# lowc1012/tensorflow-distributed-example

Hardware: AMD Instinct MI355X
Metric: images/sec (whole node) MNIST CNN at 1/2/4/8 MI355X; step time ms (higher is better)
Workload: dtype fp32; 1 GPU; model=mnist_cnn, global_batch=64, per_gpu_batch=64, parallelism=dp1, replicas=1, replicas_per_process=1, distinct_devices=1, graphs_per_execution=1, steps_per_execution=3, warmup_steps_run=6783, optimizer=SGD(lr=0.001), plan=fused_convnet, allreduce=none, hipgraph=True, grad_buckets=1, optimizer_placement=in_step_kernels

## Files before the change

### csrc/include/tde_convnet.h

```cpp
#pragma once
#include "tde_optim.h"
#include "tde_xgmi.h"

namespace tde {
namespace cnet {

constexpr int CC = 32;
constexpr int HD = 64;
constexpr int NW = 16;

struct FwdArgs {
  const float* x; const float* wc; const float* bc;
  const void* W1; int ldw1;
  float* hpre;
  void* Pt; int ldPt;
  uint64_t* amax; int lda;
  int B, H, W;
  long long* stamps;
  int w1_rows;
  const int* pend;
  const float *gwc, *gbc, *mwc, *mbc, *vwc, *vbc;
  const long long* iterations;
  OptHyper h;
  unsigned long long* inc_iter;
// ... 137 lines not shown
    for (int t = 0; t < 9; ++t) {
      wlo[t] = *reinterpret_cast<const float4*>(wcs + t * CC + c0);
      whi[t] = *reinterpret_cast<const float4*>(wcs + t * CC + c0 + 4);
    }
    blo = *reinterpret_cast<const float4*>(wcs + 9 * CC + c0);
    bhi = *reinterpret_cast<const float4*>(wcs + 9 * CC + c0 + 4);
  }
};

__device__ __forceinline__ float f4get(float4 q, int k) { return k == 0 ? q.x : (k == 1 ? q.y : (k == 2 ? q.z : q.w)); }

__device__ __forceinline__ void conv_pool8(const float* xb, int W, const ConvW8& cw, float out[8], uint64_t& packed) {
  float patch[16];
#pragma unroll
  for (int r = 0; r < 4; ++r) {
    const float2 u = *reinterpret_cast<const float2*>(xb + r * W);
    const float2 v = *reinterpret_cast<const float2*>(xb + r * W + 2);
    patch[r * 4 + 0] = u.x; patch[r * 4 + 1] = u.y; patch[r * 4 + 2] = v.x; patch[r * 4 + 3] = v.y;
  }
  packed = 0;
#pragma unroll
  for (int cc = 0; cc < 8; ++cc) {
    float wt[9];
#pragma unroll
    for (int t = 0; t < 9; ++t) wt[t] = f4get(cc < 4 ? cw.wlo[t] : cw.whi[t], cc & 3);
    const float bcv = f4get(cc < 4 ? cw.blo : cw.bhi, cc & 3);
    float best = -3.0e38f;
    int bi = 0;
#pragma unroll
    for (int q = 0; q < 4; ++q) {
      const int dy = q >> 1, dx = q & 1;
      float z = bcv;
#pragma unroll
      for (int ky = 0; ky < 3; ++ky)
#pragma unroll
        for (int kx = 0; kx < 3; ++kx) z = fmaf(patch[(dy + ky) * 4 + dx + kx], wt[ky * 3 + kx], z);
      if (z > best) { best = z; bi = q; }
    }
    out[cc] = fmaxf(best, 0.f);
    packed |= (uint64_t)(best > 0.f ? (unsigned)bi : 0xFFu) << (8 * cc);
  }
}

struct BwdArgs {
  const float* x; const uint64_t* amax; int lda;
  const float* hpre;
  float* hzero;
  int hrep; long long hrep_stride;
  float* cpart;
  const float* b1; const float* W2; const float* b2; int C; int pre_relu;
  const int* labels;
  float scale;
  float* metrics;
  const void* W1; int ldw1;
  const void* Pt; int ldPt;
  float* dW1;
  float* dwc; float* dbc;
  int crep; long long crep_stride;
  float *dW2, *db2, *db1;
  int B, H, W;
  long long* stamps;
  float *w1, *m1, *v1;
  bf16* w1r_out;
  bf16* w1c_out; int ldw1c;
  float *hw, *hm, *hv;
  long long off_w2, off_b2, off_b1;
  const long long* iterations;
  long long* iter_prev;
  OptHyper h;
  FlatApply commit;
  int* pend_set;
  XgPush push;
};

template <int NPER>
struct FlatPrefetch {
  int e[NPER];
  float w[NPER], g[NPER], m[NPER], v[NPER];
  __device__ __forceinline__ void load(const FlatApply& f, int tid, int nt) {
#pragma unroll
    for (int k = 0; k < NPER; ++k) {
      int idx = tid + k * nt;
      e[k] = -1;
      for (int r = 0; r < f.nr; ++r) {
        if (idx < f.n[r]) {
          e[k] = f.lo[r] + idx;
          break;
        }
        idx -= f.n[r];
      }
      w[k] = g[k] = m[k] = v[k] = 0.f;
      if (e[k] >= 0) {
        w[k] = f.w[e[k]];
        g[k] = flat_grad(f, e[k]);
        if (opt_has_m(f.h.kind)) m[k] = f.m[e[k]];
        if (opt_has_v(f.h.kind)) v[k] = f.v[e[k]];
      }
    }
  }
  __device__ __forceinline__ void apply(const FlatApply& f, long long t) {
    const float lr_t = opt_lr_t(f.h, t);
#pragma unroll
    for (int k = 0; k < NPER; ++k) {
      if (e[k] < 0) continue;
      f.w[e[k]] = opt_step(f.h, lr_t, w[k], g[k], m[k], v[k]);
      flat_grad_zero(f, e[k]);
      if (opt_has_m(f.h.kind)) f.m[e[k]] = m[k];
      if (opt_has_v(f.h.kind)) f.v[e[k]] = v[k];
    }
  }
};

__device__ __forceinline__ f32x4 mfma_f32x4(float a, float b, f32x4 c) {
  return __builtin_amdgcn_mfma_f32_16x16x4f32(a, b, c, 0, 0, 0);
}

constexpr int HS = HD + 4;
constexpr int DLS = 17, W2S = 17;
constexpr int kHeadScratch = 64 * HS * 4 + 12 * 64 * 4 * 4 + 64 * DLS * 4;
struct HeadLds {
  float* hs;
  float* part;
  float* dls;
  float* w2s;
  float* b2s;
  int* labs;
  __device__ __forceinline__ static HeadLds carve(unsigned char* scratch, unsigned char* w2, unsigned char* b2,
                                                  unsigned char* lab) {
    HeadLds l;
    l.hs = reinterpret_cast<float*>(scratch);
    l.part = reinterpret_cast<float*>(scratch + 64 * HS * 4);
    l.dls = reinterpret_cast<float*>(scratch + 64 * HS * 4 + 12 * 64 * 4 * 4);
    l.w2s = reinterpret_cast<float*>(w2);
    l.b2s = reinterpret_cast<float*>(b2);
    l.labs = reinterpret_cast<int*>(lab);
    return l;
  }
};
constexpr int kW2Bytes = HD * W2S * 4, kB2Bytes = 16 * 4, kLabBytes = 64 * 4;

__device__ __forceinline__ void head_load_w2(const BwdArgs& a, const HeadLds& l, int tid) {
  const int u = tid >> 4, c = tid & 15;
  l.w2s[u * W2S + c] = c < a.C ? a.W2[u * a.C + c] : 0.f;
  if (tid < 16) l.b2s[tid] = tid < a.C ? a.b2[tid] : 0.f;
}

__device__ __forceinline__ void zero_other_parity(const BwdArgs& a, int tid) {
  const int n4 = (int)(((a.hrep - 1) * a.hrep_stride + (long long)a.B * HD) / 4);
  const int per = (n4 + gridDim.x - 1) / gridDim.x, beg = blockIdx.x * per;
  const int end = min(n4, beg + per);
  for (int i = beg + tid; i < end; i += 1024) reinterpret_cast<float4*>(a.hzero)[i] = float4{0.f, 0.f, 0.f, 0.f};
}

__device__ __forceinline__ int opaque_tid() {
  int t = threadIdx.x;
  asm volatile("" : "+v"(t));
  return t;
}

constexpr int kMaxRep = 8;
template <int N>
struct HpreRep {
  float4 v[N];
  __device__ __forceinline__ void issue(const BwdArgs& a, int row, int c4) {
#pragma unroll
    for (int r = 0; r < N; ++r)
      v[r] = *reinterpret_cast<const float4*>(a.hpre + (size_t)min(r, a.hrep - 1) * a.hrep_stride + (size_t)row * HD + c4);
  }
  __device__ __forceinline__ float4 sum(const BwdArgs& a) const {
    float4 s = v[0];
#pragma unroll
    for (int r = 1; r < N; ++r) {
      const bool on = r < a.hrep;
      s.x += on ? v[r].x : 0.f; s.y += on ? v[r].y : 0.f; s.z += on ? v[r].z : 0.f; s.w += on ? v[r].w : 0.f;
    }
    return s;
  }
};
__device__ __forceinline__ float4 load_hpre_loop(const BwdArgs& a, int row, int c4) {
  float4 s = {0.f, 0.f, 0.f, 0.f};
  for (int r = 0; r < a.hrep; ++r) {
    const float4 v = *reinterpret_cast<const float4*>(a.hpre + (size_t)r * a.hrep_stride + (size_t)row * HD + c4);
    s.x += v.x; s.y += v.y; s.z += v.z; s.w += v.w;
  }
  return s;
}
template <int N>
__device__ __forceinline__ float4 load_hpre_n(const BwdArgs& a, int row, int c4) {
  HpreRep<N> h;
  h.issue(a, row, c4);
  return h.sum(a);
}
__device__ __forceinline__ float4 load_hpre_sw(const BwdArgs& a, int row, int c4) {
  if (a.hrep > kMaxRep) return load_hpre_loop(a, row, c4);
  switch (a.hrep) {
    case 1: return load_hpre_n<1>(a, row, c4);
    case 2: return load_hpre_n<2>(a, row, c4);
    case 3: case 4: return load_hpre_n<4>(a, row, c4);
    default: return load_hpre_n<8>(a, row, c4);
  }
}
__device__ __forceinline__ float4 load_hpre(const BwdArgs& a, int row, int c4) {
  if (a.hrep > kMaxRep) return load_hpre_loop(a, row, c4);
  float4 v[kMaxRep];
#pragma unroll
  for (int r = 0; r < kMaxRep; ++r)
    v[r] = r < a.hrep ? *reinterpret_cast<const float4*>(a.hpre + (size_t)r * a.hrep_stride + (size_t)row * HD + c4)
                      : float4{0.f, 0.f, 0.f, 0.f};
  float4 s = v[0];
#pragma unroll
  for (int r = 1; r < kMaxRep; ++r) {
    s.x += v[r].x; s.y += v[r].y; s.z += v[r].z; s.w += v[r].w;
  }
  return s;
}

__device__ __forceinline__ void head_stage(const BwdArgs& a, float4 hv, float4 b1v, int hr, int hc4, int nb,
                                           float* hs) {
  float4 h = float4{hv.x + b1v.x, hv.y + b1v.y, hv.z + b1v.z, hv.w + b1v.w};
  if (a.pre_relu) h = float4{fmaxf(h.x, 0.f), fmaxf(h.y, 0.f), fmaxf(h.z, 0.f), fmaxf(h.w, 0.f)};
  if (hr >= nb) h = float4{0.f, 0.f, 0.f, 0.f};
  *reinterpret_cast<float4*>(hs + hr * HS + hc4) = h;
}

__device__ __forceinline__ void head_logits_ce(const BwdArgs& a, int nb, const HeadLds& l, int lane, int wave,
                                               float& la, float& ca, float& na) {
  const int fr = lane & 15, fq = lane >> 4, C = a.C;
  f32x4 lg = {0.f, 0.f, 0.f, 0.f};
  {
    const int rt = wave & 3, kq = wave >> 2;
#pragma unroll
    for (int k = kq * 16; k < kq * 16 + 16; k += 4)
      lg = mfma_f32x4(l.hs[(rt * 16 + fr) * HS + k + fq], l.w2s[(k + fq) * W2S + fr], lg);
    if (kq > 0) *reinterpret_cast<f32x4*>(l.part + (((kq - 1) * 4 + rt) * 64 + lane) * 4) = lg;
  }
  lds_barrier();
  if (wave < 4) {
    const int rt = wave;
#pragma unroll
    for (int q = 0; q < 3; ++q) {
      const f32x4 pv = *reinterpret_cast<const f32x4*>(l.part + ((q * 4 + rt) * 64 + lane) * 4);
      lg[0] += pv[0]; lg[1] += pv[1]; lg[2] += pv[2]; lg[3] += pv[3];
    }
#pragma unroll
    for (int i = 0; i < 4; ++i) {
      const int r = rt * 16 + fq * 4 + i;
      const bool valid = r < nb;
      const bool cv = fr < C;
      const float z = cv ? lg[i] + l.b2s[fr] : -3.0e38f;
      const float m = row16_max(z);
      const float e = cv ? __expf(z - m) : 0.f;
      const float s = row16_sum(e);
      const float pr = e / s;
      const int label = l.labs[r];
      const int amx = row16_min(cv && z == m ? fr : 64);
      const float zl = __shfl(z, (lane & ~15) | (label & 15), 64);
      if (valid && fr == 0) {
        la += __logf(s) + m - zl;
        ca += (amx == label) ? 1.f : 0.f;
        na += 1.f;
      }
      l.dls[r * DLS + fr] = (valid && cv) ? (pr - (fr == label ? 1.f : 0.f)) * a.scale : 0.f;
    }
  }
  lds_barrier();
}

__device__ __forceinline__ f32x4 head_dh(const BwdArgs& a, int nb, const HeadLds& l, int lane, int wave) {
  const int fr = lane & 15, fq = lane >> 4, rt = wave >> 2, ut = wave & 3;
  f32x4 gh = {0.f, 0.f, 0.f, 0.f};
#pragma unroll
  for (int k = 0; k < 16; k += 4)
    gh = mfma_f32x4(l.dls[(rt * 16 + fr) * DLS + k + fq], l.w2s[(ut * 16 + fr) * W2S + k + fq], gh);
  const int j = ut * 16 + fr;
#pragma unroll
  for (int i = 0; i < 4; ++i) {
    const int r = rt * 16 + fq * 4 + i;
    if ((a.pre_relu && !(l.hs[r * HS + j] > 0.f)) || r >= nb) gh[i] = 0.f;
  }
  return gh;
}

__device__ __forceinline__ long long head_var(const BwdArgs& a, int tid, int i) {
  const int lane = tid & 63, wave = tid >> 6, fr = lane & 15, fq = lane >> 4, C = a.C;
  if (wave < 4 && fr < C) return a.off_w2 + (long long)(wave * 16 + fq * 4 + i) * C + fr;
  if (i == 0 && wave == 4 && fq == 0 && fr < C) return a.off_b2 + fr;
  if (i == 0 && wave == 5 && a.off_b1 >= 0) return a.off_b1 + lane;
  return -1;
}

template <int MODE, bool LEAN = false>
__device__ __forceinline__ void head_workgroup(const BwdArgs& a, const HeadLds& l, float* db1p) {
  const int lane = threadIdx.x & 63, wave = threadIdx.x >> 6, tid = threadIdx.x;
  const int fr = lane & 15, fq = lane >> 4, C = a.C;
  const float4 b1v = a.b1 ? *reinterpret_cast<const float4*>(a.b1 + (tid & 15) * 4) : float4{0.f, 0.f, 0.f, 0.f};

  float hwv[4] = {0.f, 0.f, 0.f, 0.f}, hmv[4] = {0.f, 0.f, 0.f, 0.f}, hvv[4] = {0.f, 0.f, 0.f, 0.f};
  long long t_it = 0;
  FlatPrefetch<1> cp;
  int cpend = 0;
  if (MODE != 0) {
    t_it = *a.iterations;
    const int tl = LEAN ? opaque_tid() : (int)threadIdx.x;
#pragma unroll
    for (int i = 0; i < 4; ++i) {
      const long long e = head_var(a, tl, i);
      if (e < 0) continue;
      hwv[i] = a.hw[e];
      if (MODE == 2 && opt_has_m(a.h.kind)) hmv[i] = a.hm[e];
      if (MODE == 2 && opt_has_v(a.h.kind)) hvv[i] = a.hv[e];
    }
    if (a.commit.nr > 0) {
      cpend = *a.commit.pend;
      cp.load(a.commit, tid, 1024);
    }
  }

  f32x4 gw = {0.f, 0.f, 0.f, 0.f};
  float db1acc = 0.f, db2acc = 0.f, la = 0.f, ca = 0.f, na = 0.f;
  for (int b0 = 0; b0 < a.B; b0 += 64) {
    const int nb = min(64, a.B - b0);
    const int tid = LEAN ? opaque_tid() : (int)threadIdx.x;
    const int lane = tid & 63, wave = tid >> 6, fr = lane & 15, fq = lane >> 4;
    const int hr = tid >> 4, hc4 = (tid & 15) * 4;
    float4 hv = {0.f, 0.f, 0.f, 0.f};
    if (hr < nb) hv = LEAN ? load_hpre_sw(a, b0 + hr, hc4) : load_hpre(a, b0 + hr, hc4);
    const int lab = (tid < nb) ? a.labels[b0 + tid] : 0;
    head_stage(a, hv, b1v, hr, hc4, nb, l.hs);
    if (tid < 64) l.labs[tid] = lab;
    lds_barrier();
    head_logits_ce(a, nb, l, lane, wave, la, ca, na);
    const f32x4 gh = head_dh(a, nb, l, lane, wave);
    db1acc += (gh[0] + gh[1]) + (gh[2] + gh[3]);
    if (wave < 4) {
#pragma unroll
      for (int k = 0; k < 64; k += 4) gw = mfma_f32x4(l.hs[(k + fq) * HS + wave * 16 + fr], l.dls[(k + fq) * DLS + fr], gw);
    } else if (wave == 4) {
#pragma unroll 4
      for (int r = fq * 16; r < fq * 16 + 16; ++r) db2acc += l.dls[r * DLS + fr];
    }
    lds_barrier();
  }
  db1acc += __shfl_xor(db1acc, 16, 64);
  db1acc += __shfl_xor(db1acc, 32, 64);
  if (fq == 0) db1p[(wave >> 2) * 64 + (wave & 3) * 16 + fr] = db1acc;
  db2acc += __shfl_xor(db2acc, 16, 64);
  db2acc += __shfl_xor(db2acc, 32, 64);
  if (wave < 4) {
    la = rows4_sum(la);
    ca = rows4_sum(ca);
    na = rows4_sum(na);
    if (a.metrics && lane == 0 && na > 0.f) {
      atomicAdd(a.metrics + 0, la);
      atomicAdd(a.metrics + 1, ca);
      atomicAdd(a.metrics + 2, na);
    }
  }
  lds_barrier();
  float gv[4] = {0.f, 0.f, 0.f, 0.f};
  float* gdst[4] = {nullptr, nullptr, nullptr, nullptr};
  if (wave < 4 && fr < C) {
#pragma unroll
    for (int i = 0; i < 4; ++i) {
      gv[i] = gw[i];
      gdst[i] = a.dW2 ? a.dW2 + (size_t)(wave * 16 + fq * 4 + i) * C + fr : nullptr;
    }
  } else if (wave == 4 && fq == 0 && fr < C) {
    gv[0] = db2acc;
    gdst[0] = a.db2 ? a.db2 + fr : nullptr;
  } else if (wave == 5 && a.b1) {
    gv[0] = (db1p[lane] + db1p[64 + lane]) + (db1p[128 + lane] + db1p[192 + lane]);
    gdst[0] = a.db1 ? a.db1 + lane : nullptr;
  }
  if (MODE == 0) {
#pragma unroll
    for (int i = 0; i < 4; ++i)
      if (gdst[i]) *gdst[i] += gv[i];
    stamp(a.stamps, 7);
    return;
  }
  const float lr_t = opt_lr_t(a.h, t_it);
  const int tl = LEAN ? opaque_tid() : (int)threadIdx.x;
#pragma unroll
  for (int i = 0; i < 4; ++i) {
    const long long e = head_var(a, tl, i);
    if (e < 0) continue;
    float m = hmv[i], v = hvv[i];
    a.hw[e] = opt_step(a.h, lr_t, hwv[i], gv[i], m, v);
    if (MODE == 2 && opt_has_m(a.h.kind)) a.hm[e] = m;
    if (MODE == 2 && opt_has_v(a.h.kind)) a.hv[e] = v;
  }
  if (cpend) cp.apply(a.commit, t_it - 1);
  if (tid == 0) {
    if (cpend) *a.commit.pend = 0;
    if (cpend && a.commit.count) atomicAdd(a.commit.count, 1ull);
    if (a.pend_set) *a.pend_set = 1;
    if (a.iter_prev) *a.iter_prev = t_it;
  }
  stamp(a.stamps, 7);
}

__device__ __forceinline__ void conv_grad_reduce(const BwdArgs& a, const f32x4 accr[2], float* red, int lane, int wave) {
  const int fr = lane & 15, fq = lane >> 4, tid = threadIdx.x;
#pragma unroll
  for (int ct = 0; ct < 2; ++ct)
#pragma unroll
    for (int r = 0; r < 4; ++r) red[((size_t)wave * 16 + fq * 4 + r) * CC + ct * 16 + fr] = accr[ct][r];
  lds_barrier();
  if (tid < 10 * CC) {
    const int tap = tid / CC, c = tid - tap * CC;
    float s = 0.f;
#pragma unroll
    for (int w = 0; w < NW; ++w) s += red[((size_t)w * 16 + tap) * CC + c];
    if (a.cpart) a.cpart[(size_t)blockIdx.x * 10 * CC + tid] = s;
    else {
      const long long ro = a.crep > 1 ? (long long)(blockIdx.x % a.crep) * a.crep_stride : 0;
      if (tap < 9) {
        if (a.dwc) atomicAdd(a.dwc + ro + tap * CC + c, s);
      } else if (a.dbc) {
        atomicAdd(a.dbc + ro + c, s);
      }
    }
  }
}

}
}


struct TdeStepOpt {
  tde::OptHyper h;
  float *w, *g, *m, *v;
  const long long* iterations;
  int* pend;
  int grep; long long grep_stride;
  unsigned long long* fly_count;
  const float *hsrc_w2, *hsrc_b2, *hsrc_b1;
  float* hsnap;
  int hC;
};

struct TdeBwdOpt {
  tde::OptHyper h;
  float *w, *m, *v;
  long long off_w1, off_w2, off_b2, off_b1;
  void* W1c; int ldw1c;
  const long long* iterations;
  long long* iter_prev;
  tde::FlatApply commit;
  int* pend_set;
  int crep; long long crep_stride;
};

namespace tde {
namespace cnet {

inline bool opt_ok(const TdeStepOpt* o) {
  return opt_kind_fused(o->h.kind) && o->w && o->g && o->iterations && opt_slots_ok(o->h.kind, o->m, o->v) &&
         (!o->hsnap || (o->hsrc_w2 && o->hsrc_b2 && o->hC >= 1 && o->hC <= 16 && !((uintptr_t)o->hsnap & 15)));
}

inline void fill_fwd_opt(FwdArgs& a, const TdeStepOpt* opt, long long off_wc, long long off_bc, long long* inc_iter,
                         int hrep, long long hrep_stride) {
  a.inc_iter = (unsigned long long*)inc_iter;
  a.hrep = hrep > 0 ? hrep : 1;
  a.hrep_stride = hrep_stride;
  if (opt) {
    a.pend = opt->pend;
    a.gwc = opt->g + off_wc;
    a.gbc = opt->g + off_bc;
    a.mwc = opt->m ? opt->m + off_wc : nullptr;
    a.mbc = opt->m ? opt->m + off_bc : nullptr;
    a.vwc = opt->v ? opt->v + off_wc : nullptr;
    a.vbc = opt->v ? opt->v + off_bc : nullptr;
    a.iterations = opt->iterations;
    a.h = opt->h;
    a.grep = opt->grep > 1 ? opt->grep : 1;
    a.grep_stride = opt->grep_stride;
    a.fly_count = opt->fly_count;
    a.hsrc_w2 = opt->hsrc_w2;
    a.hsrc_b2 = opt->hsrc_b2;
    a.hsrc_b1 = opt->hsrc_b1;
    a.hsnap = opt->hsnap;
    a.hC = opt->hC;
  } else {
    a.grep = 1;
    a.grep_stride = 0;
  }
}

inline int fill_bwd(BwdArgs& a, const float* x, const void* amax, int lda, const float* hpre, float* hzero, int hrep,
                    long long hrep_stride, const float* b1, const float* W2, const float* b2, int C, int pre_relu,
                    const int* labels, float scale, float* metrics, const void* W1, int ldw1, const void* Pt, int ldPt,
                    float* dW1, float* dwc, float* dbc, float* dW2, float* db2, float* db1, int B, int H, int W,
                    long long* stamps, const TdeBwdOpt* opt) {
  if ((ldw1 & 7) || (ldPt & 7) || ldPt < B || lda < B || C < 1 || C > 16 || !hpre || !hzero || !labels) return -1;
  if ((((uintptr_t)hpre | (uintptr_t)hzero | (uintptr_t)b1) & 15)) return -2;
  if (opt && (!opt_kind_fused(opt->h.kind) || (opt->commit.nr > 0 && !opt_kind_fused(opt->commit.h.kind)) || !opt->w || !opt->iterations ||
              !opt_slots_ok(opt->h.kind, opt->m, opt->v) ||
              ldw1 != HD || (opt->W1c && (opt->ldw1c & 3)) || (opt->off_w1 & 3) || opt->commit.nr > kFlatRanges ||
              (opt->commit.nr > 0 && !opt->commit.pend) || (b1 != nullptr) != (opt->off_b1 >= 0)))
    return -4;
  if (opt && opt->commit.nr > 0) {
    int total = 0;
    for (int i = 0; i < opt->commit.nr; ++i) total += opt->commit.n[i];
    if (total > 1024) return -5;
  }
  if (hrep < 1 || hrep > 1024 || (hrep > 1 && (hrep_stride < (long long)B * HD || (hrep_stride & 3)))) return -6;
  a = BwdArgs{};
  a.x = x;
  a.amax = (const uint64_t*)amax;
// ... 55 lines not shown
```

### csrc/kernels/convnet_f32.hip

```cpp
#include "tde_convnet.h"

namespace tde {
using namespace cnet;

constexpr int FG = 4;
constexpr int FB = 16;
constexpr int AS32 = 168;
constexpr int GS32 = 72;
constexpr int DPS32 = 40;
static_assert(FG == 4 && FB == 16, "the forward's lane maps are written for 4 positions x 16 images");

__host__ __device__ constexpr int fwd32_istride(int W) { return XR * W + ((4 - (XR * W) % 64) + 64) % 64; }
constexpr int kXr32Bytes = FB * (XR * XW + 64) * 4;
constexpr int kFwd32Lds = FB * AS32 * 4 + kXr32Bytes + kConvW * 4;

__device__ __forceinline__ int k8_col(int fq, int i) { return fq * 8 + 4 * ((i + fq) & 1); }
__device__ __forceinline__ int k16_col(int fq, int i) { return fq * 16 + 4 * ((i + fq) & 3); }

struct Fwd32X {
  static constexpr int kU = 3;
  static_assert(FB * XR * XW / 4 <= kU * 256, "one pass of the workgroup stages the rows");
  float4 v[kU];
  __device__ __forceinline__ void issue(const FwdArgs& a, int b0, int py0, int nrows) {
    const int W = a.W, H = a.H;
    const int n4 = nrows * W / 4;
#pragma unroll
    for (int u = 0; u < kU; ++u) {
      const int i = threadIdx.x + u * 256, bl = i / n4, q = i - bl * n4;
      v[u] = float4{0.f, 0.f, 0.f, 0.f};
      if (i < FB * n4 && b0 + bl < a.B)
        v[u] = *reinterpret_cast<const float4*>(a.x + (size_t)(b0 + bl) * H * W + (size_t)(2 * py0) * W + q * 4);
    }
  }
  __device__ __forceinline__ void store(const FwdArgs& a, float* xr, int nrows) const {
    const int W = a.W;
    const int istride = fwd32_istride(W);
    const int n4 = nrows * W / 4;
#pragma unroll
    for (int u = 0; u < kU; ++u) {
      const int i = threadIdx.x + u * 256, bl = i / n4, q = i - bl * n4;
      if (i < FB * n4) *reinterpret_cast<float4*>(xr + bl * istride + q * 4) = v[u];
    }
  }
};

__global__ __launch_bounds__(256) void convnet32_fwd_kernel(FwdArgs a) {
  constexpr int NT = 256;
  extern __shared__ __attribute__((aligned(16))) unsigned char fsm[];
  float* As = reinterpret_cast<float*>(fsm);
  float* xr = reinterpret_cast<float*>(fsm + FB * AS32 * 4);
  float* wcs = reinterpret_cast<float*>(fsm + FB * AS32 * 4 + kXr32Bytes);
  int pendv;
  long long iterv;
  conv_flags_issue(a, pendv, iterv);
  stamp(a.stamps, 0);
  if (a.inc_iter && blockIdx.x == 0 && blockIdx.y == 0 && threadIdx.x == 0) atomicAdd(a.inc_iter, 1ull);
  const int lane = threadIdx.x & 63, wave = __builtin_amdgcn_readfirstlane(threadIdx.x >> 6);
  const int fr = lane & 15, fq = lane >> 4;
  const int W = a.W, H = a.H;
  const int Wp = (W - 2) / 2, Hp = (H - 2) / 2, P = Hp * Wp;
  const int p0 = blockIdx.x * FG;
  const int b0 = blockIdx.y * FB;
  const int py0 = p0 / Wp;
  const int nrows = min(XR, H - 2 * py0);
  const float* W1 = reinterpret_cast<const float*>(a.W1);
  float* Pt = reinterpret_cast<float*>(a.Pt);

  static_assert(kConvW > NT && kConvW <= NT + 64, "wave 0 holds the conv operands past the first NT");
  Fwd32X xst;
  xst.issue(a, b0, py0, nrows);
  ConvOperand cv0, cv1;
  cv0.issue(a, threadIdx.x);
  if (wave == 0) cv1.issue(a, NT + min((int)threadIdx.x, kConvW - NT - 1));
  SnapHead<NT> snap;
  const bool snap_wg = SnapHead<NT>::mine(a);
  if (snap_wg) snap.issue(a);
  const int nt = wave;
  float wfr[FG][8];
#pragma unroll
  for (int ks = 0; ks < FG; ++ks) {
    const int kp = min(p0 + ks, P - 1);
#pragma unroll
    for (int i = 0; i < 2; ++i)
#pragma unroll
      for (int j = 0; j < 4; ++j) wfr[ks][4 * i + j] = W1[(size_t)(kp * CC + k8_col(fq, i) + j) * a.ldw1 + nt * 16 + fr];
  }
  xst.store(a, xr, nrows);
  wcs[threadIdx.x] = cv0.finish(a, pendv, iterv);
  if (wave == 0 && threadIdx.x < kConvW - NT) wcs[NT + threadIdx.x] = cv1.finish(a, pendv, iterv);
  if (snap_wg) snap.store(a);
  if (a.fly_count && pendv && blockIdx.x == 0 && blockIdx.y == 0 && threadIdx.x == 0) atomicAdd(a.fly_count, 1ull);
  stamp(a.stamps, 1);
  lds_barrier();

  const int cg = wave, c0 = cg * 8;
  ConvW8 cw;
  cw.load(wcs, c0);
  const int p = p0 + fq, b = b0 + fr;
  const bool pok = p < P, bok = b < a.B;
  float out[8];
  if (bok && pok) {
    const int py = p / Wp, px = p - py * Wp;
    uint64_t packed;
    conv_pool8(xr + fr * fwd32_istride(W) + (2 * (py - py0)) * W + 2 * px, W, cw, out, packed);
    if (a.amax) a.amax[((size_t)p * (CC / 8) + cg) * a.lda + b] = packed;
  } else {
#pragma unroll
    for (int cc = 0; cc < 8; ++cc) out[cc] = 0.f;
  }
  if (pok && Pt && (bok || b < a.ldPt)) {
#pragma unroll
    for (int cc = 0; cc < 8; ++cc) Pt[(size_t)(p * CC + c0 + cc) * a.ldPt + b] = out[cc];
  }
  {
    float* dst = As + fr * AS32 + fq * CC + c0;
    *reinterpret_cast<float4*>(dst) = float4{out[0], out[1], out[2], out[3]};
    *reinterpret_cast<float4*>(dst + 4) = float4{out[4], out[5], out[6], out[7]};
  }
  stamp(a.stamps, 2);
  lds_barrier();
  stamp(a.stamps, 3);

#pragma unroll
  for (int ks = 0; ks < FG; ++ks)
#pragma unroll
    for (int i = 0; i < 8; ++i) wfr[ks][i] = p0 + ks < P ? wfr[ks][i] : 0.f;
  float* const hrow = a.hpre + (size_t)(blockIdx.x % a.hrep) * a.hrep_stride;
  f32x4 acc[FG];
#pragma unroll
  for (int ks = 0; ks < FG; ++ks) acc[ks] = f32x4{0.f, 0.f, 0.f, 0.f};
#pragma unroll
  for (int i = 0; i < 2; ++i) {
    float4 av[FG];
#pragma unroll
    for (int ks = 0; ks < FG; ++ks)
      av[ks] = *reinterpret_cast<const float4*>(As + fr * AS32 + ks * CC + k8_col(fq, i));
#pragma unroll
    for (int e = 0; e < 4; ++e)
#pragma unroll
      for (int ks = 0; ks < FG; ++ks) acc[ks] = mfma_f32x4(f4get(av[ks], e), wfr[ks][4 * i + e], acc[ks]);
  }
#pragma unroll
  for (int r = 0; r < 4; ++r) {
    const int row = b0 + fq * 4 + r;
    const float s = ((acc[0][r] + acc[1][r]) + acc[2][r]) + acc[3][r];
    if (row < a.B) atomicAdd(hrow + (size_t)row * HD + nt * 16 + fr, s);
  }
  stamp(a.stamps, 4);
}

constexpr int kG32 = 0;
constexpr int kGt32 = kG32 + 64 * GS32 * 4;
constexpr int kW1s32 = kGt32 + 64 * GS32 * 4;
constexpr int kPts32 = kW1s32 + 32 * GS32 * 4;
constexpr int kXs32 = kPts32 + 32 * GS32 * 4;
constexpr int kAm32 = kXs32 + 64 * 16 * 4;
constexpr int kR32 = kAm32 + 64 * CC;
constexpr int kRBytes = kHeadScratch > NW * 16 * CC * 4 ? kHeadScratch : NW * 16 * CC * 4;
static_assert(64 * DPS32 * 4 <= kRBytes, "dP exceeds the shared scratch");
constexpr int kW2s32 = kR32 + kRBytes;
constexpr int kB2s32 = kW2s32 + kW2Bytes;
constexpr int kLab32 = kB2s32 + kB2Bytes;
constexpr int kBwd32Lds = kLab32 + kLabBytes;
static_assert(kBwd32Lds <= 160 * 1024, "backward LDS exceeds a CU");

__device__ __forceinline__ void bwd32_ids(int& tid, int& lane, int& wave, int& fr, int& fq) {
  const int t = opaque_tid();
  tid = t;
  lane = t & 63;
  wave = t >> 6;
  fr = lane & 15;
  fq = lane >> 4;
}

struct Bwd32Chunk {
  float4 hv;
  int lab;
  float2 ptv;
  float4 xv;
  uint64_t amv;
};

template <int NREP>
__device__ __forceinline__ void bwd32_chunk_issue(const BwdArgs& a, int tid, int p, int py, int px, int b0, int nb,
                                                  Bwd32Chunk& c) {
  const int last = nb - 1;
  const int hrow = b0 + min(tid >> 4, last), hc4 = (tid & 15) * 4;
  HpreRep<(NREP > 0 ? NREP : 1)> h;
  if (NREP > 0) h.issue(a, hrow, hc4);
  c.lab = a.labels[b0 + min(tid, last)];
  const int pc = (tid & 31) * 2;
  c.ptv = *reinterpret_cast<const float2*>(reinterpret_cast<const float*>(a.Pt) + (size_t)(p * CC + (tid >> 5)) * a.ldPt +
                                           b0 + min(pc, last & ~1));
  c.xv = float4{0.f, 0.f, 0.f, 0.f};
  c.amv = ~0ull;
  if (tid < 256) {
    const int bl = tid >> 2, r = tid & 3;
    const float2* row = reinterpret_cast<const float2*>(a.x + (size_t)(b0 + min(bl, last)) * a.H * a.W +
                                                        (2 * py + r) * a.W + 2 * px);
    const float2 u = row[0], t = row[1];
    c.xv = float4{u.x, u.y, t.x, t.y};
    const int cg = tid >> 6, bb = tid & 63;
    c.amv = a.amax[((size_t)p * (CC / 8) + cg) * a.lda + b0 + min(bb, last)];
  }
  c.hv = NREP > 0 ? h.sum(a) : load_hpre_loop(a, hrow, hc4);
  if ((tid >> 2) >= nb) c.xv = float4{0.f, 0.f, 0.f, 0.f};
  if ((tid & 63) >= nb) c.amv = ~0ull;
  if (tid >= nb) c.lab = 0;
  if (pc >= nb) c.ptv.x = 0.f;
  if (pc + 1 >= nb) c.ptv.y = 0.f;
}

template <int MODE>
__global__ __launch_bounds__(1024) void convnet32_bwd_kernel(BwdArgs a) {
  extern __shared__ __attribute__((aligned(16))) unsigned char smem[];
  float* Gs = reinterpret_cast<float*>(smem + kG32);
  float* Gts = reinterpret_cast<float*>(smem + kGt32);
  float* W1s = reinterpret_cast<float*>(smem + kW1s32);
  float* Pts = reinterpret_cast<float*>(smem + kPts32);
  float* xs = reinterpret_cast<float*>(smem + kXs32);
  uint8_t* am = smem + kAm32;
  float* dps = reinterpret_cast<float*>(smem + kR32);
  const HeadLds hl = HeadLds::carve(smem + kR32, smem + kW2s32, smem + kB2s32, smem + kLab32);
  long long t_it = 0;
  if (MODE == 2) t_it = *a.iterations;
  const unsigned nwg = gridDim.x;
  stamp(a.stamps, 0);
  const int W = a.W;
  int tid, lane, wave, fr, fq;
  bwd32_ids(tid, lane, wave, fr, fq);
  const float* W1 = reinterpret_cast<const float*>(a.W1);

  float w2v, b2v;
  {
    const int u2 = tid >> 4, c2 = tid & 15;
    w2v = a.W2[u2 * a.C + min(c2, a.C - 1)];
    b2v = a.b2[min(c2, a.C - 1)];
  }
  zero_other_parity(a, tid);
  if (blockIdx.x == nwg - 1) {
    hl.w2s[(tid >> 4) * W2S + (tid & 15)] = (tid & 15) < a.C ? w2v : 0.f;
    if (tid < 16) hl.b2s[tid] = tid < a.C ? b2v : 0.f;
    head_workgroup<MODE, true>(a, hl, Gs);
    return;
  }

  const int Wp = (W - 2) / 2;
  const int p = blockIdx.x;
  const int py = p / Wp, px = p - py * Wp;
  const float4 b1v = *reinterpret_cast<const float4*>((a.b1 ? a.b1 : a.hpre) + (tid & 15) * 4);
  f32x4 accw = {0.f, 0.f, 0.f, 0.f};
  f32x4 accr[2] = {{0.f, 0.f, 0.f, 0.f}, {0.f, 0.f, 0.f, 0.f}};

  f32x4 mp = {0.f, 0.f, 0.f, 0.f}, vp = {0.f, 0.f, 0.f, 0.f};
  if (MODE == 2 && wave >= 8) {
    const int rt = (wave & 7) >> 2, nt = wave & 3;
#pragma unroll
    for (int r = 0; r < 4; ++r) {
      const size_t e = (size_t)(p * CC + rt * 16 + fq * 4 + r) * HD + nt * 16 + fr;
      if (opt_has_m(a.h.kind)) mp[r] = a.m1[e];
      if (opt_has_v(a.h.kind)) vp[r] = a.v1[e];
    }
  }

  const float2 w1v = *reinterpret_cast<const float2*>(W1 + (size_t)(p * CC + (tid >> 5)) * a.ldw1 + (tid & 31) * 2);

  for (int b0 = 0; b0 < a.B; b0 += 64) {
    const int nb = min(64, a.B - b0);
    bwd32_ids(tid, lane, wave, fr, fq);
    const bool dw_wave = wave >= 8;
    const int v8 = wave & 7;
    Bwd32Chunk ck;
    if (a.hrep > kMaxRep) bwd32_chunk_issue<0>(a, tid, p, py, px, b0, nb, ck);
    else switch (a.hrep) {
      case 1: bwd32_chunk_issue<1>(a, tid, p, py, px, b0, nb, ck); break;
      case 2: bwd32_chunk_issue<2>(a, tid, p, py, px, b0, nb, ck); break;
      case 3: case 4: bwd32_chunk_issue<4>(a, tid, p, py, px, b0, nb, ck); break;
      default: bwd32_chunk_issue<8>(a, tid, p, py, px, b0, nb, ck); break;
    }
    stamp(a.stamps, 1);
    const bool has_b1 = a.b1 && tid >= 0;
    const float4 b1u = has_b1 ? b1v : float4{0.f, 0.f, 0.f, 0.f};
    if (b0 == 0) {
      hl.w2s[(tid >> 4) * W2S + (tid & 15)] = (tid & 15) < a.C ? w2v : 0.f;
      if (tid < 16) hl.b2s[tid] = tid < a.C ? b2v : 0.f;
      *reinterpret_cast<float2*>(W1s + (tid >> 5) * GS32 + (tid & 31) * 2) = w1v;
    }
    head_stage(a, ck.hv, b1u, tid >> 4, (tid & 15) * 4, nb, hl.hs);
    if (tid < 64) hl.labs[tid] = ck.lab;
    *reinterpret_cast<float2*>(Pts + (tid >> 5) * GS32 + (tid & 31) * 2) = ck.ptv;
    if (tid < 256) {
      const int bl = tid >> 2, r = tid & 3;
      *reinterpret_cast<float4*>(xs + bl * 16 + r * 4) = ck.xv;
      const int cg = tid >> 6, bb = tid & 63;
      *reinterpret_cast<uint64_t*>(am + bb * CC + cg * 8) = ck.amv;
    }
    lds_barrier();
    {
      float la = 0.f, ca = 0.f, na = 0.f;
      head_logits_ce(a, nb, hl, lane, wave, la, ca, na);
      const f32x4 gh = head_dh(a, nb, hl, lane, wave);
      const int rt = wave >> 2, j = (wave & 3) * 16 + fr;
#pragma unroll
      for (int i = 0; i < 4; ++i) Gs[(rt * 16 + fq * 4 + i) * GS32 + j] = gh[i];
      *reinterpret_cast<float4*>(Gts + j * GS32 + rt * 16 + fq * 4) = float4{gh[0], gh[1], gh[2], gh[3]};
    }
    lds_barrier();
    stamp(a.stamps, 2);

    {
      const float* Ab = dw_wave ? Pts + ((v8 >> 2) * 16 + fr) * GS32 : Gs + ((v8 >> 1) * 16 + fr) * GS32;
      const float* Bb = dw_wave ? Gts + ((v8 & 3) * 16 + fr) * GS32 : W1s + ((v8 & 1) * 16 + fr) * GS32;
      f32x4 acc = dw_wave ? accw : f32x4{0.f, 0.f, 0.f, 0.f};
#pragma unroll
      for (int i = 0; i < 4; ++i) {
        const float4 av = *reinterpret_cast<const float4*>(Ab + k16_col(fq, i));
        const float4 bv = *reinterpret_cast<const float4*>(Bb + k16_col(fq, i));
        acc = mfma_f32x4(av.x, bv.x, acc);
        acc = mfma_f32x4(av.y, bv.y, acc);
        acc = mfma_f32x4(av.z, bv.z, acc);
        acc = mfma_f32x4(av.w, bv.w, acc);
      }
      if (dw_wave) {
        accw = acc;
      } else {
        const int mt = v8 >> 1, ct = v8 & 1;
#pragma unroll
        for (int r = 0; r < 4; ++r) dps[(mt * 16 + fq * 4 + r) * DPS32 + ct * 16 + fr] = acc[r];
      }
    }
    lds_barrier();
    stamp(a.stamps, 3);

    {
      const int tap = fr, ky = tap / 3, kx = tap - ky * 3, qy = fq >> 1, qx = fq & 1;
#pragma unroll
      for (int s = 0; s < 4; ++s) {
        const int bl = wave * 4 + s;
        const float xa = tap < 9 ? xs[bl * 16 + (qy + ky) * 4 + qx + kx] : (tap == 9 ? 1.f : 0.f);
#pragma unroll
        for (int ct = 0; ct < 2; ++ct) {
          const int c = ct * 16 + fr;
          const float d = am[bl * CC + c] == (unsigned)fq ? dps[bl * DPS32 + c] : 0.f;
          accr[ct] = mfma_f32x4(xa, d, accr[ct]);
        }
      }
    }
    lds_barrier();
  }
  stamp(a.stamps, 4);

  bwd32_ids(tid, lane, wave, fr, fq);
  const bool dw_wave = wave >= 8;
  const int v8 = wave & 7;
  if (dw_wave) {
    const int rt = v8 >> 2, nt = v8 & 3;
    const int col = nt * 16 + fr;
    if (MODE != 0) {
      const float lr_t = opt_lr_t(a.h, t_it);
#pragma unroll
      for (int r = 0; r < 4; ++r) {
        const int row = rt * 16 + fq * 4 + r;
        const size_t e = (size_t)(p * CC + row) * HD + col;
        float m = mp[r], v = vp[r];
        a.w1[e] = opt_step(a.h, lr_t, W1s[row * GS32 + col], accw[r], m, v);
        if (MODE == 2 && opt_has_m(a.h.kind)) a.m1[e] = m;
        if (MODE == 2 && opt_has_v(a.h.kind)) a.v1[e] = v;
      }
    } else if (a.push.nranks > 0) {
#pragma unroll
      for (int r = 0; r < 4; ++r) W1s[(rt * 16 + fq * 4 + r) * GS32 + col] = accw[r];
    } else {
#pragma unroll
      for (int r = 0; r < 4; ++r) a.dW1[(size_t)(p * CC + rt * 16 + fq * 4 + r) * HD + col] = accw[r];
    }
  }
  conv_grad_reduce(a, accr, dps, lane, wave);
  if (MODE == 0 && a.push.nranks > 0 && tid < CC * HD / 4) {
    const int parity = (int)((*a.push.epoch + 1u) & 1u);
    const int row = tid >> 4, c4 = (tid & 15) * 4;
    xg_push_store4(a.push, parity, a.push.off + (long long)(p * CC + row) * HD + c4,
                   *reinterpret_cast<const float4*>(W1s + row * GS32 + c4));
    xg_push_drain();
  }
  stamp(a.stamps, 5);
}

}

using namespace tde;
using namespace tde::cnet;

TDE_API int tde_convnet_fwd_f32(const float* x, const float* wc, const float* bc, const float* W1, int ldw1,
                                float* hpre, float* Pt, int ldPt, void* amax, int lda, int B, int H, int W,
                                long long* stamps, const TdeStepOpt* opt, long long off_wc, long long off_bc,
                                long long* inc_iter, int hrep, long long hrep_stride, hipStream_t stream) {
  if ((W & 3) || W > XW || ((W - 2) / 2) < 4 || ldw1 != HD || (Pt && (ldPt & 7)) || (amax && lda < B)) return -1;
  if (((uintptr_t)wc | (uintptr_t)bc | (uintptr_t)W1) & 15) return -2;
  if (opt && (!opt_ok(opt) || !opt->pend)) return -4;
  const int P = ((H - 2) / 2) * ((W - 2) / 2);
  const int by = ((Pt && ldPt > B ? ldPt : B) + FB - 1) / FB;
  FwdArgs a{x, wc, bc, W1, ldw1, hpre, Pt, ldPt, (uint64_t*)amax, lda, B, H, W, stamps};
  fill_fwd_opt(a, opt, off_wc, off_bc, inc_iter, hrep, hrep_stride);
  const dim3 grid((P + FG - 1) / FG, by);
  convnet32_fwd_kernel<<<grid, 256, kFwd32Lds, stream>>>(a);
  TDE_LAUNCH_CHECK();
  return 0;
}

TDE_API int tde_convnet_bwd_f32(const float* x, const void* amax, int lda, const float* hpre, float* hzero,
                                int hrep, long long hrep_stride, const float* b1, const float* W2, const float* b2,
                                int C, int pre_relu, const int* labels, float scale, float* metrics, const float* W1,
                                int ldw1, const float* Pt, int ldPt, float* dW1, float* dwc, float* dbc, float* dW2,
                                float* db2, float* db1, int B, int H, int W, long long* stamps, const TdeBwdOpt* opt,
                                float* cpart, const XgPush* push, int crep, long long crep_stride,
                                hipStream_t stream) {
  if (ldw1 != HD || ((uintptr_t)W1 & 15) || ((uintptr_t)Pt & 7)) return -1;
  if (push && push->nranks > 0 &&
      (opt || push->nranks > kXgMaxRanks || push->L <= 0 || (push->L & 3) || (push->off & 3) || !push->epoch))
    return -7;
  if (opt && opt->w + opt->off_w1 != W1) return -3;
  BwdArgs a;
  const int rc = fill_bwd(a, x, amax, lda, hpre, hzero, hrep, hrep_stride, b1, W2, b2, C, pre_relu, labels, scale,
                          metrics, W1, ldw1, Pt, ldPt, dW1, dwc, dbc, dW2, db2, db1, B, H, W, stamps, opt);
  if (rc) return rc;
  a.cpart = cpart;
  a.w1r_out = nullptr;
  a.w1c_out = nullptr;
  if (push) a.push = *push;
  if (!opt && crep > 1) {
    a.crep = crep;
    a.crep_stride = crep_stride;
  }
  const int P = ((H - 2) / 2) * ((W - 2) / 2);
  static bool attr_set = false;
  if (!attr_set) {
    (void)hipFuncSetAttribute((const void*)convnet32_bwd_kernel<0>, hipFuncAttributeMaxDynamicSharedMemorySize, kBwd32Lds);
    (void)hipFuncSetAttribute((const void*)convnet32_bwd_kernel<1>, hipFuncAttributeMaxDynamicSharedMemorySize, kBwd32Lds);
    (void)hipFuncSetAttribute((const void*)convnet32_bwd_kernel<2>, hipFuncAttributeMaxDynamicSharedMemorySize, kBwd32Lds);
    attr_set = true;
  }
  const dim3 grid(P + 1);
  if (!opt) convnet32_bwd_kernel<0><<<grid, 1024, kBwd32Lds, stream>>>(a);
  else if (opt->h.kind == kOptSGD) convnet32_bwd_kernel<1><<<grid, 1024, kBwd32Lds, stream>>>(a);
  else convnet32_bwd_kernel<2><<<grid, 1024, kBwd32Lds, stream>>>(a);
  TDE_LAUNCH_CHECK();
  return 0;
}

TDE_API int tde_cnet_abi_sizes(long long* out, int n) {
  const long long s[] = {(long long)sizeof(TdeStepOpt), (long long)sizeof(TdeBwdOpt), (long long)sizeof(FlatApply),
                         (long long)sizeof(OptHyper)};
  for (int i = 0; i < n && i < 4; ++i) out[i] = s[i];
  return 4;
}
```

Before: 2.776 million images/sec.

## Split head logits across all waves and specialize backward kernel for 28x28

Adds a head logits path in which all 16 waves each compute a K-quarter of the logits MFMA. The partial sums are written to LDS and reduced before the softmax/CE, instead of a few waves doing the full K loop. The fused backward body is templated on a compile-time geometry so the 28x28 MNIST case gets constant H/W/ldw1 and a constant workgroup count, with a runtime switch to fall back. It also moves the lean path's metric atomics to one per workgroup and adds fine-grained timestamp probes. The cost is extra LDS barriers and partial-sum traffic.

```diff
diff --git a/csrc/include/tde_convnet.h b/csrc/include/tde_convnet.h
--- a/csrc/include/tde_convnet.h
+++ b/csrc/include/tde_convnet.h
@@ -313,6 +313,13 @@
   for (int i = beg + tid; i < end; i += 1024) reinterpret_cast<float4*>(a.hzero)[i] = float4{0.f, 0.f, 0.f, 0.f};
 }
 
+__device__ __forceinline__ void zero_other_parity_n(const BwdArgs& a, int tid, int nwg) {
+  const int n4 = (int)(((a.hrep - 1) * a.hrep_stride + (long long)a.B * HD) / 4);
+  const int per = (n4 + nwg - 1) / nwg, beg = blockIdx.x * per;
+  const int end = min(n4, beg + per);
+  for (int i = beg + tid; i < end; i += 1024) reinterpret_cast<float4*>(a.hzero)[i] = float4{0.f, 0.f, 0.f, 0.f};
+}
+
 __device__ __forceinline__ int opaque_tid() {
   int t = threadIdx.x;
   asm volatile("" : "+v"(t));
@@ -427,6 +434,57 @@
   lds_barrier();
 }
 
+__device__ __forceinline__ void stamp_fine(long long* st, int slot) {
+  if (st && threadIdx.x == 0) {
+    asm volatile("s_waitcnt lgkmcnt(0)" ::: "memory");
+    st[(size_t)(gridDim.x + blockIdx.x) * kMaxStamps + slot - kMaxStamps] = (long long)__builtin_amdgcn_s_memrealtime();
+  }
+}
+
+template <bool METRICS>
+__device__ __forceinline__ void head_logits_ce16(const BwdArgs& a, int nb, const HeadLds& l, float* part0, int lane,
+                                                 int wave, float& la, float& ca, float& na) {
+  const int fr = lane & 15, fq = lane >> 4, C = a.C;
+  {
+    const int rt = wave & 3, kq = wave >> 2;
+    f32x4 lg = {0.f, 0.f, 0.f, 0.f};
+#pragma unroll
+    for (int k = kq * 16; k < kq * 16 + 16; k += 4)
+      lg = mfma_f32x4(l.hs[(rt * 16 + fr) * HS + k + fq], l.w2s[(k + fq) * W2S + fr], lg);
+    float* dst = (kq == 0 ? part0 : l.part + (kq - 1) * 1024) + rt * 256 + lane;
+#pragma unroll
+    for (int i = 0; i < 4; ++i) dst[i * 64] = lg[i];
+  }
+  lds_barrier();
+  stamp_fine(a.stamps, 10);
+  {
+    const int rt = wave & 3, i = wave >> 2;
+    const int o = rt * 256 + i * 64 + lane;
+    const float p0 = part0[o], p1 = l.part[o], p2 = l.part[1024 + o], p3 = l.part[2048 + o];
+    const float lgi = ((p0 + p1) + p2) + p3;
+    const int r = rt * 16 + fq * 4 + i;
+    const bool valid = r < nb;
+    const bool cv = fr < C;
+    const float z = cv ? lgi + l.b2s[fr] : -3.0e38f;
+    const float m = row16_max(z);
+    const float e = cv ? __expf(z - m) : 0.f;
+    const float s = row16_sum(e);
+    const float pr = e / s;
+    const int label = l.labs[r];
+    if (METRICS) {
+      const int amx = row16_min(cv && z == m ? fr : 64);
+      const float zl = __shfl(z, (lane & ~15) | (label & 15), 64);
+      if (valid && fr == 0) {
+        la += __logf(s) + m - zl;
+        ca += (amx == label) ? 1.f : 0.f;
+        na += 1.f;
+      }
+    }
+    l.dls[r * DLS + fr] = (valid && cv) ? (pr - (fr == label ? 1.f : 0.f)) * a.scale : 0.f;
+  }
+  lds_barrier();
+}
+
 __device__ __forceinline__ f32x4 head_dh(const BwdArgs& a, int nb, const HeadLds& l, int lane, int wave) {
   const int fr = lane & 15, fq = lane >> 4, rt = wave >> 2, ut = wave & 3;
   f32x4 gh = {0.f, 0.f, 0.f, 0.f};
@@ -490,7 +548,8 @@
     head_stage(a, hv, b1v, hr, hc4, nb, l.hs);
     if (tid < 64) l.labs[tid] = lab;
     lds_barrier();
-    head_logits_ce(a, nb, l, lane, wave, la, ca, na);
+    if (LEAN) head_logits_ce16<true>(a, nb, l, db1p, lane, wave, la, ca, na);
+    else head_logits_ce(a, nb, l, lane, wave, la, ca, na);
     const f32x4 gh = head_dh(a, nb, l, lane, wave);
     db1acc += (gh[0] + gh[1]) + (gh[2] + gh[3]);
     if (wave < 4) {
@@ -507,7 +566,16 @@
   if (fq == 0) db1p[(wave >> 2) * 64 + (wave & 3) * 16 + fr] = db1acc;
   db2acc += __shfl_xor(db2acc, 16, 64);
   db2acc += __shfl_xor(db2acc, 32, 64);
-  if (wave < 4) {
+  if (LEAN) {
+    la = rows4_sum(la);
+    ca = rows4_sum(ca);
+    na = rows4_sum(na);
+    if (lane == 0) {
+      db1p[256 + wave * 4 + 0] = la;
+      db1p[256 + wave * 4 + 1] = ca;
+      db1p[256 + wave * 4 + 2] = na;
+    }
+  } else if (wave < 4) {
     la = rows4_sum(la);
     ca = rows4_sum(ca);
     na = rows4_sum(na);
@@ -518,6 +586,20 @@
     }
   }
   lds_barrier();
+  if (LEAN && a.metrics && wave == 6 && lane == 0) {
+    float ls = 0.f, cs = 0.f, ns = 0.f;
+#pragma unroll
+    for (int w = 0; w < NW; ++w) {
+      ls += db1p[256 + w * 4 + 0];
+      cs += db1p[256 + w * 4 + 1];
+      ns += db1p[256 + w * 4 + 2];
+    }
+    if (ns > 0.f) {
+      atomicAdd(a.metrics + 0, ls);
+      atomicAdd(a.metrics + 1, cs);
+      atomicAdd(a.metrics + 2, ns);
+    }
+  }
   float gv[4] = {0.f, 0.f, 0.f, 0.f};
   float* gdst[4] = {nullptr, nullptr, nullptr, nullptr};
   if (wave < 4 && fr < C) {
diff --git a/csrc/kernels/convnet_f32.hip b/csrc/kernels/convnet_f32.hip
--- a/csrc/kernels/convnet_f32.hip
+++ b/csrc/kernels/convnet_f32.hip
@@ -16,6 +16,14 @@
 
 __device__ __forceinline__ int k8_col(int fq, int i) { return fq * 8 + 4 * ((i + fq) & 1); }
 __device__ __forceinline__ int k16_col(int fq, int i) { return fq * 16 + 4 * ((i + fq) & 3); }
+
+template <int GH, int GW>
+struct Geo {
+  static constexpr bool kFixed = GH > 0;
+  template <class A> __device__ __forceinline__ static int H(const A& a) { return kFixed ? GH : a.H; }
+  template <class A> __device__ __forceinline__ static int W(const A& a) { return kFixed ? GW : a.W; }
+};
+constexpr int kGH = 28, kGW = 28;
 
 struct Fwd32X {
   static constexpr int kU = 3;
@@ -181,7 +189,14 @@
   uint64_t amv;
 };
 
-template <int NREP>
+__device__ __forceinline__ void stamp_landed(long long* st, const Bwd32Chunk& c) {
+  if (st) {
+    asm volatile("" ::"v"(c.hv.x), "v"(c.lab), "v"(c.ptv.x), "v"(c.xv.x), "v"((int)c.amv));
+    stamp_fine(st, 8);
+  }
+}
+
+template <int NREP, class G>
 __device__ __forceinline__ void bwd32_chunk_issue(const BwdArgs& a, int tid, int p, int py, int px, int b0, int nb,
                                                   Bwd32Chunk& c) {
   const int last = nb - 1;
@@ -196,8 +211,8 @@
   c.amv = ~0ull;
   if (tid < 256) {
     const int bl = tid >> 2, r = tid & 3;
-    const float2* row = reinterpret_cast<const float2*>(a.x + (size_t)(b0 + min(bl, last)) * a.H * a.W +
-                                                        (2 * py + r) * a.W + 2 * px);
+    const float2* row = reinterpret_cast<const float2*>(a.x + (size_t)(b0 + min(bl, last)) * G::H(a) * G::W(a) +
+                                                        (2 * py + r) * G::W(a) + 2 * px);
     const float2 u = row[0], t = row[1];
     c.xv = float4{u.x, u.y, t.x, t.y};
     const int cg = tid >> 6, bb = tid & 63;
@@ -211,9 +226,8 @@
   if (pc + 1 >= nb) c.ptv.y = 0.f;
 }
 
-template <int MODE>
-__global__ __launch_bounds__(1024) void convnet32_bwd_kernel(BwdArgs a) {
-  extern __shared__ __attribute__((aligned(16))) unsigned char smem[];
+template <int MODE, class G>
+__device__ __forceinline__ void convnet32_bwd_body(const BwdArgs& a, unsigned char* smem) {
   float* Gs = reinterpret_cast<float*>(smem + kG32);
   float* Gts = reinterpret_cast<float*>(smem + kGt32);
   float* W1s = reinterpret_cast<float*>(smem + kW1s32);
@@ -224,9 +238,9 @@
   const HeadLds hl = HeadLds::carve(smem + kR32, smem + kW2s32, smem + kB2s32, smem + kLab32);
   long long t_it = 0;
   if (MODE == 2) t_it = *a.iterations;
-  const unsigned nwg = gridDim.x;
+  const unsigned nwg = G::kFixed ? ((kGH - 2) / 2) * ((kGW - 2) / 2) + 1 : gridDim.x;
   stamp(a.stamps, 0);
-  const int W = a.W;
+  const int W = G::W(a);
   int tid, lane, wave, fr, fq;
   bwd32_ids(tid, lane, wave, fr, fq);
   const float* W1 = reinterpret_cast<const float*>(a.W1);
@@ -237,7 +251,7 @@
     w2v = a.W2[u2 * a.C + min(c2, a.C - 1)];
     b2v = a.b2[min(c2, a.C - 1)];
   }
-  zero_other_parity(a, tid);
+  zero_other_parity_n(a, tid, (int)nwg);
   if (blockIdx.x == nwg - 1) {
     hl.w2s[(tid >> 4) * W2S + (tid & 15)] = (tid & 15) < a.C ? w2v : 0.f;
     if (tid < 16) hl.b2s[tid] = tid < a.C ? b2v : 0.f;
@@ -263,7 +277,7 @@
     }
   }
 
-  const float2 w1v = *reinterpret_cast<const float2*>(W1 + (size_t)(p * CC + (tid >> 5)) * a.ldw1 + (tid & 31) * 2);
+  const float2 w1v = *reinterpret_cast<const float2*>(W1 + (size_t)(p * CC + (tid >> 5)) * (G::kFixed ? HD : a.ldw1) + (tid & 31) * 2);
 
   for (int b0 = 0; b0 < a.B; b0 += 64) {
     const int nb = min(64, a.B - b0);
@@ -271,14 +285,15 @@
     const bool dw_wave = wave >= 8;
     const int v8 = wave & 7;
     Bwd32Chunk ck;
-    if (a.hrep > kMaxRep) bwd32_chunk_issue<0>(a, tid, p, py, px, b0, nb, ck);
+    if (a.hrep > kMaxRep) bwd32_chunk_issue<0, G>(a, tid, p, py, px, b0, nb, ck);
     else switch (a.hrep) {
-      case 1: bwd32_chunk_issue<1>(a, tid, p, py, px, b0, nb, ck); break;
-      case 2: bwd32_chunk_issue<2>(a, tid, p, py, px, b0, nb, ck); break;
-      case 3: case 4: bwd32_chunk_issue<4>(a, tid, p, py, px, b0, nb, ck); break;
-      default: bwd32_chunk_issue<8>(a, tid, p, py, px, b0, nb, ck); break;
+      case 1: bwd32_chunk_issue<1, G>(a, tid, p, py, px, b0, nb, ck); break;
+      case 2: bwd32_chunk_issue<2, G>(a, tid, p, py, px, b0, nb, ck); break;
+      case 3: case 4: bwd32_chunk_issue<4, G>(a, tid, p, py, px, b0, nb, ck); break;
+      default: bwd32_chunk_issue<8, G>(a, tid, p, py, px, b0, nb, ck); break;
     }
     stamp(a.stamps, 1);
+    stamp_landed(a.stamps, ck);
     const bool has_b1 = a.b1 && tid >= 0;
     const float4 b1u = has_b1 ? b1v : float4{0.f, 0.f, 0.f, 0.f};
     if (b0 == 0) {
@@ -296,14 +311,17 @@
       *reinterpret_cast<uint64_t*>(am + bb * CC + cg * 8) = ck.amv;
     }
     lds_barrier();
+    stamp_fine(a.stamps, 9);
     {
       float la = 0.f, ca = 0.f, na = 0.f;
-      head_logits_ce(a, nb, hl, lane, wave, la, ca, na);
+      head_logits_ce16<false>(a, nb, hl, Gs, lane, wave, la, ca, na);
+      stamp_fine(a.stamps, 11);
       const f32x4 gh = head_dh(a, nb, hl, lane, wave);
       const int rt = wave >> 2, j = (wave & 3) * 16 + fr;
 #pragma unroll
       for (int i = 0; i < 4; ++i) Gs[(rt * 16 + fq * 4 + i) * GS32 + j] = gh[i];
       *reinterpret_cast<float4*>(Gts + j * GS32 + rt * 16 + fq * 4) = float4{gh[0], gh[1], gh[2], gh[3]};
+      stamp_fine(a.stamps, 12);
     }
     lds_barrier();
     stamp(a.stamps, 2);
@@ -386,10 +404,29 @@
   stamp(a.stamps, 5);
 }
 
+template <int MODE>
+__global__ __launch_bounds__(1024) void convnet32_bwd_kernel(BwdArgs a) {
+  extern __shared__ __attribute__((aligned(16))) unsigned char smem[];
+  convnet32_bwd_body<MODE, Geo<0, 0>>(a, smem);
+}
+template <int MODE>
+__global__ __launch_bounds__(1024) void convnet32g_bwd_kernel(BwdArgs a) {
+  extern __shared__ __attribute__((aligned(16))) unsigned char smem[];
+  convnet32_bwd_body<MODE, Geo<kGH, kGW>>(a, smem);
+}
+
 }
 
 using namespace tde;
 using namespace tde::cnet;
+
+static int g_runtime_geom = 0;
+static bool geom_fixed(int H, int W) { return !g_runtime_geom && H == kGH && W == kGW; }
+TDE_API int tde_convnet_f32_runtime_geom(int on) {
+  const int prev = g_runtime_geom;
+  g_runtime_geom = on ? 1 : 0;
+  return prev;
+}
 
 TDE_API int tde_convnet_fwd_f32(const float* x, const float* wc, const float* bc, const float* W1, int ldw1,
                                 float* hpre, float* Pt, int ldPt, void* amax, int lda, int B, int H, int W,
@@ -438,12 +475,22 @@
     (void)hipFuncSetAttribute((const void*)convnet32_bwd_kernel<0>, hipFuncAttributeMaxDynamicSharedMemorySize, kBwd32Lds);
     (void)hipFuncSetAttribute((const void*)convnet32_bwd_kernel<1>, hipFuncAttributeMaxDynamicSharedMemorySize, kBwd32Lds);
     (void)hipFuncSetAttribute((const void*)convnet32_bwd_kernel<2>, hipFuncAttributeMaxDynamicSharedMemorySize, kBwd32Lds);
+    (void)hipFuncSetAttribute((const void*)convnet32g_bwd_kernel<0>, hipFuncAttributeMaxDynamicSharedMemorySize, kBwd32Lds);
+    (void)hipFuncSetAttribute((const void*)convnet32g_bwd_kernel<1>, hipFuncAttributeMaxDynamicSharedMemorySize, kBwd32Lds);
+    (void)hipFuncSetAttribute((const void*)convnet32g_bwd_kernel<2>, hipFuncAttributeMaxDynamicSharedMemorySize, kBwd32Lds);
     attr_set = true;
   }
   const dim3 grid(P + 1);
-  if (!opt) convnet32_bwd_kernel<0><<<grid, 1024, kBwd32Lds, stream>>>(a);
-  else if (opt->h.kind == kOptSGD) convnet32_bwd_kernel<1><<<grid, 1024, kBwd32Lds, stream>>>(a);
-  else convnet32_bwd_kernel<2><<<grid, 1024, kBwd32Lds, stream>>>(a);
+  const int mode = !opt ? 0 : (opt->h.kind == kOptSGD ? 1 : 2);
+  if (geom_fixed(H, W)) {
+    if (mode == 0) convnet32g_bwd_kernel<0><<<grid, 1024, kBwd32Lds, stream>>>(a);
+    else if (mode == 1) convnet32g_bwd_kernel<1><<<grid, 1024, kBwd32Lds, stream>>>(a);
+    else convnet32g_bwd_kernel<2><<<grid, 1024, kBwd32Lds, stream>>>(a);
+  } else {
+    if (mode == 0) convnet32_bwd_kernel<0><<<grid, 1024, kBwd32Lds, stream>>>(a);
+    else if (mode == 1) convnet32_bwd_kernel<1><<<grid, 1024, kBwd32Lds, stream>>>(a);
+    else convnet32_bwd_kernel<2><<<grid, 1024, kBwd32Lds, stream>>>(a);
+  }
   TDE_LAUNCH_CHECK();
   return 0;
 }
```

Measured after the change: 2.821 million images/sec (median of 6 runs). 1.6% higher.
